# ml-jku/LaM-SLidE

Measured on AMD Instinct MI355X. Metric: sampled trajectories/sec (50-step ODE) + decoded-coord L2 vs ref, MD17, higher is better.
Workload: dtype bf16; 1 GPU; md17_bench; tail=False, ln_fuse=True, T=30, L=256, C=32, D=512, H=16, depth=4, sampler=ODE, state_updates=50, batch_per_gpu=32, global_batch=32, parallelism=batch-shard x1, 1 gather to rank 0 per step, noise_elem_stride_per_rank=7864320, kernels=general, trajectories_per_pass=32

## Files before the change

### lam_slide_amd/csrc/common.hip.h

```cpp
#pragma once
#include <hip/hip_runtime.h>
#include <stdint.h>

typedef unsigned short u16;
typedef __attribute__((ext_vector_type(8))) __bf16 bf16x8;
typedef __attribute__((ext_vector_type(4))) __bf16 bf16x4;
typedef __attribute__((ext_vector_type(16))) float f32x16;
typedef __attribute__((ext_vector_type(4))) short s16x4;
typedef __attribute__((ext_vector_type(4))) unsigned int u32x4;
typedef __attribute__((ext_vector_type(2))) unsigned int u32x2;

#define LDS_PTR(T) __attribute__((address_space(3))) T *

#define LSL_PROBE(v, bit) ((v) & (bit))

template <int N>
__device__ __forceinline__ void wait_vmcnt() { asm volatile("s_waitcnt vmcnt(%0)" ::"n"(N) : "memory"); }

__device__ __forceinline__ const char *uni_ptr(const char *q) {
    const unsigned long long v = (unsigned long long)q;
    const unsigned lo32 = __builtin_amdgcn_readfirstlane((unsigned)v), hi32 = __builtin_amdgcn_readfirstlane((unsigned)(v >> 32));
    return reinterpret_cast<const char *>(((unsigned long long)hi32 << 32) | lo32);
}
__device__ __forceinline__ void lds_dma16(unsigned voff, const void *base, unsigned dst) {
    asm volatile("s_mov_b32 m0, %2\n\ts_nop 4\n\tglobal_load_lds_dwordx4 %0, %1" ::"v"(voff), "s"(base), "s"(dst) : "memory");
}

__device__ __forceinline__ f32x16 mfma32(bf16x8 a, bf16x8 b, f32x16 c) {
    return __builtin_amdgcn_mfma_f32_32x32x16_bf16(a, b, c, 0, 0, 0);
}

__device__ __forceinline__ int acc_row(int reg, int hf) { return (reg & 3) + 8 * (reg >> 2) + 4 * hf; }

__device__ __forceinline__ u16 f2bf(float f) {
    __bf16 b = (__bf16)f;
    return __builtin_bit_cast(u16, b);
}
__device__ __forceinline__ float bf2f(u16 v) { return __uint_as_float(((unsigned)v) << 16); }

typedef __attribute__((ext_vector_type(2))) __bf16 bf16x2;
typedef __attribute__((ext_vector_type(2))) float f32x2;
__device__ __forceinline__ unsigned pack2(float lo, float hi) {
    const f32x2 v = {lo, hi};
    return __builtin_bit_cast(unsigned, __builtin_convertvector(v, bf16x2));
}

__device__ __forceinline__ bf16x8 as_bf16x8(u32x4 v) { return __builtin_bit_cast(bf16x8, v); }
__device__ __forceinline__ u32x4 as_u32x4(bf16x8 v) { return __builtin_bit_cast(u32x4, v); }

__device__ __forceinline__ float wave_sum(float v) {
#pragma unroll
    for (int o = 32; o > 0; o >>= 1) v += __shfl_xor(v, o, 64);
    return v;
}

#define LSL_DPP_ADD(v, ctrl, rows) ((v) + __builtin_bit_cast(float, __builtin_amdgcn_update_dpp(0, __builtin_bit_cast(int, (v)), (ctrl), (rows), 0xF, false)))
__device__ __forceinline__ float wave_sum_dpp(float v) {
    v = LSL_DPP_ADD(v, 0x111, 0xF);
    v = LSL_DPP_ADD(v, 0x112, 0xF);
    v = LSL_DPP_ADD(v, 0x114, 0xF);
    v = LSL_DPP_ADD(v, 0x118, 0xF);
    v = LSL_DPP_ADD(v, 0x142, 0xA);
    v = LSL_DPP_ADD(v, 0x143, 0xC);
    return __builtin_bit_cast(float, __builtin_amdgcn_readlane(__builtin_bit_cast(int, v), 63));
}
#undef LSL_DPP_ADD

__device__ __forceinline__ float xhalf(float v) { return __shfl_xor(v, 32, 64); }

__device__ __forceinline__ float half_pair_sum(float v) {
    const unsigned u = __builtin_bit_cast(unsigned, v);
    const auto p = __builtin_amdgcn_permlane32_swap(u, u, false, false);
    return __builtin_bit_cast(float, (unsigned)p[0]) + __builtin_bit_cast(float, (unsigned)p[1]);
}

__device__ __forceinline__ float quad_xor1(float v) {
    return __builtin_bit_cast(float, __builtin_amdgcn_update_dpp(0, __builtin_bit_cast(int, v), 0xB1, 0xF, 0xF, true));
}
__device__ __forceinline__ float quad_xor2(float v) {
    return __builtin_bit_cast(float, __builtin_amdgcn_update_dpp(0, __builtin_bit_cast(int, v), 0x4E, 0xF, 0xF, true));
}

__device__ __forceinline__ float oct_sum(float v) {
    v += quad_xor1(v);
    v += quad_xor2(v);
    return v + __builtin_bit_cast(float, __builtin_amdgcn_update_dpp(0, __builtin_bit_cast(int, v), 0x141, 0xF, 0xF, true));
}

__device__ __forceinline__ float silu(float x) { return x / (1.0f + __expf(-x)); }

__device__ __forceinline__ float gelu_erf(float x) { return 0.5f * x * (1.0f + erff(x * 0.70710678118654752440f)); }

#define LSL_GELU_Q(ax)                                                                                                  \
    fmaf(fmaf(fmaf(fmaf(fmaf(-0.0004733090754598379f, (ax), 0.0070845563896000385f), (ax), -0.051827382296323776f), (ax), \
                   -0.4599924385547638f), (ax), -1.1507878303527832f), (ax), -1.000037670135498f)
__device__ __forceinline__ float gelu_fast(float x) {
    const float ax = fabsf(x);
    const float h = __builtin_amdgcn_exp2f(LSL_GELU_Q(ax));
    const float relu = __builtin_amdgcn_fmed3f(x, 0.0f, __builtin_inff());
    return fmaf(-ax, h, relu);
}

__device__ __forceinline__ unsigned gelu_pair_bf16(float x0, float x1) {
    const f32x2 x = {x0, x1};
    const f32x2 ax = __builtin_elementwise_abs(x);
    f32x2 q = f32x2{-0.0004733090754598379f, -0.0004733090754598379f};
    q = __builtin_elementwise_fma(q, ax, f32x2{0.0070845563896000385f, 0.0070845563896000385f});
    q = __builtin_elementwise_fma(q, ax, f32x2{-0.051827382296323776f, -0.051827382296323776f});
    q = __builtin_elementwise_fma(q, ax, f32x2{-0.4599924385547638f, -0.4599924385547638f});
    q = __builtin_elementwise_fma(q, ax, f32x2{-1.1507878303527832f, -1.1507878303527832f});
    q = __builtin_elementwise_fma(q, ax, f32x2{-1.000037670135498f, -1.000037670135498f});
    const f32x2 h = {__builtin_amdgcn_exp2f(q[0]), __builtin_amdgcn_exp2f(q[1])};
    const f32x2 relu = {__int_as_float(max(__float_as_int(x0), 0)), __int_as_float(max(__float_as_int(x1), 0))};
    const f32x2 r = __builtin_elementwise_fma(-ax, h, relu);
    return __builtin_bit_cast(unsigned, __builtin_convertvector(r, bf16x2));
}

__device__ __forceinline__ void store16(void *p, u32x4 v, bool nt) {
    if (nt) asm volatile("global_store_dwordx4 %0, %1, off nt\n\ts_nop 1" ::"v"(p), "v"(v) : "memory");
    else *reinterpret_cast<u32x4 *>(p) = v;
}
__device__ __forceinline__ void store8(void *p, u32x2 v, bool nt) {
    if (nt) asm volatile("global_store_dwordx2 %0, %1, off nt\n\ts_nop 0" ::"v"(p), "v"(v) : "memory");
    else *reinterpret_cast<u32x2 *>(p) = v;
}

typedef __attribute__((ext_vector_type(4))) float f32x4_t;

__device__ __forceinline__ int xcd_remap(int bid, int nwg) {
    const int q = nwg >> 3, r = nwg & 7, xcd = bid & 7, idx = bid >> 3;
    const int base = xcd < r ? xcd * (q + 1) : r * (q + 1) + (xcd - r) * q;
    return base + idx;
}
```

### lam_slide_amd/csrc/k_lin1.hip.h

```cpp
#pragma once
#include <type_traits>

#include "common.hip.h"

struct Lin1Args {
    const u16 *W;
    const u16 *X;
    const float *bias;
    const float4 *rope_q, *rope_k;
    u16 *qkv;
    u16 *z;
    int F, N, HHD, M;
    int pos_div, pos_mod;
    unsigned div_magic, mod_magic;
    float inv_hd, q_premul;
    int nt;
    int wpt;
    int planes;
    int npad;
    const float2 *ln_stat;
    const float *ln_shift, *ln_scale;
    int ln_mod_stride, ln_tpt;
    unsigned ln_tpt_magic;
};

#ifndef LIN1_B2
#define LIN1_B2 1
#endif
#ifndef LIN1_B2_KMAX
#define LIN1_B2_KMAX 256
#endif

template <int HDP, int K, int NW = 8>
struct Lin1Cfg {
    static_assert(K % 128 == 0 && K <= 512, "hidden sizes 128 / 256 / 384 / 512");
    static constexpr int KS = K / 16;
    static constexpr int ROWB = 2 * K;
    static constexpr int PITCH = ROWB + 16;
    static constexpr int BLK = 32 * PITCH;
    static constexpr int NS = (LIN1_B2 && K <= LIN1_B2_KMAX) ? 4 : 3;
    static constexpr int RING = NS * BLK;
    static_assert(NW == 8 || NW == 4, "two waves per SIMD (256-token tiles) or one (128-token tiles)");
    static constexpr int TT = 32 * NW;
    static constexpr int STAGE = NW * 4096;
    static constexpr int LPR = ROWB / 16;
    static constexpr int PPW = 32 / NW;
    static constexpr size_t lds_bytes(int F) { return (size_t)RING + STAGE + (size_t)F * 4; }
    static constexpr int LN_SLOTS = K <= 256 ? 3 : 2;
    static constexpr size_t lds_bytes_lnf(int F) { return lds_bytes(F) + (size_t)LN_SLOTS * 2 * K * 4; }
};

enum { LIN1_QK = 0, LIN1_V = 1, LIN1_MLP = 2 };

#ifndef LIN1_XLOAD
#define LIN1_XLOAD 1
#endif
#ifndef LIN1_PD
#define LIN1_PD 3
#endif

__device__ __forceinline__ float lin1_gelu(float x) {
    const float ax = fabsf(x);
    const float h = __builtin_amdgcn_exp2f(LSL_GELU_Q(ax));
    float relu;
    asm("v_max_f32 %0, 0, %1" : "=v"(relu) : "v"(x));
    return fmaf(-ax, h, relu);
}

template <int HDP, int K, int NW = 8, bool LNF = false>
__global__ void __launch_bounds__(NW * 64, NW / 4) k_linear1_ts(Lin1Args g) {
    using C = Lin1Cfg<HDP, K, NW>;
    constexpr int KS = C::KS, BLK = C::BLK, PPW = C::PPW, ROWB = C::ROWB;
    constexpr int NCO = HDP == 32 ? 8 : 4;
    extern __shared__ __attribute__((aligned(16))) char smem[];

    const int tid = threadIdx.x, lane = tid & 63;
    const int wave = __builtin_amdgcn_readfirstlane(tid >> 6);
    const int r = lane & 31, hf = lane >> 5;
    char *const stage = smem + C::RING + wave * 4096;
    float *const bias_lds = reinterpret_cast<float *>(smem + C::RING + C::STAGE);

    const int NB = g.F >> 5;
    const int ntile = (g.N + C::TT - 1) / C::TT;
    const long U = (long)ntile * NB;
    long i0, i1;
    if (g.wpt > 0) {
        const int tile = blockIdx.x / g.wpt, part = blockIdx.x - tile * g.wpt;
        i0 = (long)tile * NB + ((NB * part / g.wpt) & ~1);
        i1 = (long)tile * NB + (part + 1 == g.wpt ? NB : ((NB * (part + 1) / g.wpt) & ~1));
    } else {
        i0 = (U * blockIdx.x / gridDim.x) & ~1L;
        i1 = blockIdx.x + 1 == gridDim.x ? U : ((U * (blockIdx.x + 1) / gridDim.x) & ~1L);
    }
    if (i0 >= i1) return;

    for (int i = tid * 4; i < g.F; i += NW * 64 * 4) *reinterpret_cast<float4 *>(bias_lds + i) = *reinterpret_cast<const float4 *>(g.bias + i);

    const unsigned lds0 = (unsigned)(size_t)(LDS_PTR(char))(smem);
    const unsigned lane_src = lane * 16;
    const char *const w_rows = reinterpret_cast<const char *>(g.W) + (size_t)(PPW * wave) * ROWB;
    auto issue_piece = [&](const char *src, unsigned dst, auto ic) __attribute__((always_inline)) {
        constexpr int I = decltype(ic)::value & 3;
        if (decltype(ic)::value >= 4) {
            src += 4 * ROWB;
            dst += 4 * C::PITCH;
        }
        const unsigned ls = lane_src;
        if (C::LPR == 64 || lane < C::LPR) {
            if (I == 0 || decltype(ic)::value >= 4)
                asm volatile("s_add_u32 m0, %2, %3\n\ts_nop 4\n\tglobal_load_lds_dwordx4 %0, %1 offset:%4" ::"v"(ls), "s"(src), "s"(dst), "n"(16 * I), "n"(ROWB * I) : "memory", "scc");
            else
                asm volatile("s_add_u32 m0, %2, %3\n\ts_nop 0\n\tglobal_load_lds_dwordx4 %0, %1 offset:%4" ::"v"(ls), "s"(src), "s"(dst), "n"(16 * I), "n"(ROWB * I) : "memory", "scc");
        }
    };
    auto req_src = [&](int blk) __attribute__((always_inline)) { return w_rows + (size_t)blk * (32 * ROWB); };
    auto req_dst = [&](int slot) __attribute__((always_inline)) { return lds0 + slot * BLK + PPW * wave * C::PITCH; };
    auto issue = [&](int blk, int slot) __attribute__((always_inline)) {
        const char *src = req_src(blk);
        const unsigned dst = req_dst(slot);
        issue_piece(src, dst, std::integral_constant<int, 0>());
        issue_piece(src, dst, std::integral_constant<int, 1>());
        issue_piece(src, dst, std::integral_constant<int, 2>());
        issue_piece(src, dst, std::integral_constant<int, 3>());
        if (PPW == 8) {
            issue_piece(src, dst, std::integral_constant<int, 4>());
            issue_piece(src, dst, std::integral_constant<int, 5>());
            issue_piece(src, dst, std::integral_constant<int, 6>());
            issue_piece(src, dst, std::integral_constant<int, 7>());
        }
    };
    const int aoff = r * C::PITCH + 16 * hf;

    bf16x8 xreg[KS];
    float4 co[NCO];
    f32x16 acc0, acc1;
    int slot_c = 0;
    int dma_blk, dma_slot;
    int n_wave = 0;
    float post = 1.0f;

    auto advance = [&](int &b) __attribute__((always_inline)) { b = b + 1 == NB ? 0 : b + 1; };
    auto next_slot = [&](int s) __attribute__((always_inline)) { return s == C::NS - 1 ? 0 : s + 1; };

    {
        int b = (int)(i0 - (i0 / NB) * NB);
        issue(b, 0);
        advance(b);
        issue(b, 1);
        advance(b);
        dma_blk = b;
        dma_slot = 2;
    }

    auto init_acc = [&](f32x16 &a, int blk) __attribute__((always_inline)) {
#pragma unroll
        for (int q4 = 0; q4 < 4; ++q4) {
            const float4 b = *reinterpret_cast<const float4 *>(bias_lds + blk * 32 + 8 * q4 + 4 * hf);
            a[4 * q4] = b.x; a[4 * q4 + 1] = b.y; a[4 * q4 + 2] = b.z; a[4 * q4 + 3] = b.w;
        }
    };
    constexpr bool B2 = LIN1_B2 != 0 && K <= LIN1_B2_KMAX;
    auto step_head = [&](auto flushed_c) __attribute__((always_inline)) {
        if (B2) {
            if (decltype(flushed_c)::value) wait_vmcnt<PPW>();
            else wait_vmcnt<0>();
        } else {
            if (decltype(flushed_c)::value) wait_vmcnt<2 * PPW>();
            else wait_vmcnt<PPW>();
        }
        __builtin_amdgcn_s_barrier();
        asm volatile("" ::: "memory");
    };
    const unsigned wr0 = (unsigned)(size_t)(LDS_PTR(char))(stage) + r * 128 + 8 * hf + ((r & 7) << 4);
    const unsigned rd0 = (unsigned)(size_t)(LDS_PTR(char))(stage) + (lane >> 3) * 128 + (((lane & 7) ^ ((lane >> 3) & 7)) << 4);
    const char *row_q = nullptr, *row_z = nullptr;
    const bool planes = g.planes != 0;
    constexpr unsigned PROW = 2u * HDP, CPH = HDP / 8;
    const unsigned plane_bytes = PROW * (unsigned)g.npad;
    const unsigned stride_q = planes ? PROW : 2u * 3 * g.HHD, stride_z = 2u * (g.HHD + g.M);
    const unsigned blk_q = planes ? (32 / HDP) * plane_bytes : 64u;
    const unsigned voff_q = planes ? ((lane & 7) / CPH) * plane_bytes + (lane >> 3) * PROW + 16 * ((lane & 7) % CPH) : (lane >> 3) * stride_q + 16 * (lane & 7);
    const unsigned voff_z = (lane >> 3) * stride_z + 16 * (lane & 7);
    const int slab_z = 3 * (g.HHD >> 5);
    const char *fl_base = nullptr;
    unsigned fl_stride8 = 0, fl_voff = 0;
    auto flush_setup = [&](int b_even) __attribute__((always_inline)) {
        const bool to_qkv = b_even < slab_z;
        fl_base = to_qkv ? row_q : row_z;
        fl_stride8 = 8 * (to_qkv ? stride_q : stride_z);
        fl_voff = to_qkv ? voff_q + blk_q * (unsigned)b_even : voff_z + 64u * (unsigned)b_even;
    };
    auto flush_read = [&](int half, u32x4 (&pk)[2]) __attribute__((always_inline)) {
#pragma unroll
        for (int i = 0; i < 2; ++i) pk[i] = *reinterpret_cast<const LDS_PTR(u32x4)>(rd0 + 1024 * (2 * half + i));
    };
    auto flush_store = [&](int half, const u32x4 (&pk)[2]) __attribute__((always_inline)) {
        asm volatile("s_nop 4\n\tglobal_store_dwordx4 %0, %1, %2 nt\n\ts_nop 1" ::"v"(fl_voff + (2 * half) * fl_stride8), "v"(pk[0]), "s"(fl_base) : "memory");
        asm volatile("global_store_dwordx4 %0, %1, %2 nt\n\ts_nop 1" ::"v"(fl_voff + (2 * half + 1) * fl_stride8), "v"(pk[1]), "s"(fl_base) : "memory");
    };
    auto flush_store_visible = [&](int half, const u32x4 (&pk)[2]) __attribute__((always_inline)) {
#pragma unroll
        for (int i = 0; i < 2; ++i)
            __builtin_nontemporal_store(pk[i], reinterpret_cast<u32x4 *>(const_cast<char *>(fl_base) + (size_t)(fl_voff + (2 * half + i) * fl_stride8)));
    };
    auto put_group = [&](int ii, int q, float v0, float v1, float v2, float v3) __attribute__((always_inline)) {
        const u32x2 pk = {pack2(v0, v1), pack2(v2, v3)};
        *reinterpret_cast<LDS_PTR(u32x2)>(wr0 ^ (unsigned)(64 * ii + 16 * q)) = pk;
    };
    auto epi_slice = [&](auto sec_c, int s, const f32x16 &a, int ii, float &c0, float &c1) __attribute__((always_inline)) {
        constexpr int SEC = decltype(sec_c)::value;
        if constexpr (SEC == LIN1_QK && HDP == 32) {
            if (s == 0) c0 = 0.0f;
            if (s < 2) {
#pragma unroll
                for (int e = 0; e < 8; ++e) c0 = fmaf(a[8 * s + e], a[8 * s + e], c0);
            }
            if (s == 1) c0 = rsqrtf(fmaf(half_pair_sum(c0), g.inv_hd, 1e-6f)) * post;
            if (s >= 2 && s < 6) {
                const int q = s - 2;
                float o[4];
#pragma unroll
                for (int kk = 0; kk < 2; ++kk) {
                    const int k = 2 * q + kk;
                    const float x0 = a[2 * k], x1 = a[2 * k + 1];
                    o[2 * kk] = c0 * fmaf(co[k].x, x0, -co[k].y * x1);
                    o[2 * kk + 1] = c0 * fmaf(co[k].z, x0, co[k].w * x1);
                }
                put_group(ii, q, o[0], o[1], o[2], o[3]);
            }
        } else if constexpr (SEC == LIN1_QK) {
            if (s == 0) {
                c0 = 0.0f;
#pragma unroll
                for (int e = 0; e < 8; ++e) c0 = fmaf(a[e], a[e], c0);
            }
            if (s == 1) {
                c1 = 0.0f;
#pragma unroll
                for (int e = 0; e < 8; ++e) c1 = fmaf(a[8 + e], a[8 + e], c1);
                c0 = rsqrtf(fmaf(half_pair_sum(c0), g.inv_hd, 1e-6f)) * post;
                c1 = rsqrtf(fmaf(half_pair_sum(c1), g.inv_hd, 1e-6f)) * post;
            }
            if (s >= 2 && s < 6) {
                const int q = s - 2;
                const float rr = q < 2 ? c0 : c1;
                float o[4];
#pragma unroll
                for (int kk = 0; kk < 2; ++kk) {
                    const int k = 2 * q + kk;
                    const float x0 = a[2 * k], x1 = a[2 * k + 1];
                    const float4 cf = co[k & (NCO - 1)];
                    o[2 * kk] = rr * fmaf(cf.x, x0, -cf.y * x1);
                    o[2 * kk + 1] = rr * fmaf(cf.z, x0, cf.w * x1);
                }
                put_group(ii, q, o[0], o[1], o[2], o[3]);
            }
        } else if constexpr (SEC == LIN1_MLP) {
            const float g0 = lin1_gelu(a[2 * s]), g1 = lin1_gelu(a[2 * s + 1]);
            if (s & 1) put_group(ii, s >> 1, c0, c1, g0, g1);
            else { c0 = g0; c1 = g1; }
        } else {
            if (s < 4) put_group(ii, s, a[4 * s], a[4 * s + 1], a[4 * s + 2], a[4 * s + 3]);
        }
    };
    auto step = [&](auto sec_c, auto par_c, auto mfma_c, auto epi_c, auto side) __attribute__((always_inline)) {
        constexpr int PAR = decltype(par_c)::value;
        constexpr bool DO_MFMA = decltype(mfma_c)::value != 0, DO_EPI = decltype(epi_c)::value != 0;
        constexpr int MPS = KS / 8, PD = LIN1_PD, MH = (MPS + 1) / 2;
        f32x16 &ac = PAR ? acc0 : acc1;
        const f32x16 &ae = PAR ? acc1 : acc0;
        const char *sb = smem + slot_c * BLK + aoff;
        bf16x8 fr[PD];
        float c0 = 0.0f, c1 = 0.0f;
        if (DO_MFMA) {
#pragma unroll
            for (int ks = 0; ks < PD; ++ks) fr[ks] = as_bf16x8(*reinterpret_cast<const u32x4 *>(sb + 32 * ks));
        }
        side(std::integral_constant<int, -1>());
#define LIN1_SIDE(S) if (s == S) side(std::integral_constant<int, S>());
#pragma unroll
        for (int s = 0; s < 8; ++s) {
#pragma unroll
            for (int m = 0; m < MPS; ++m) {
                if (m == MH) { LIN1_SIDE(0) LIN1_SIDE(1) LIN1_SIDE(2) LIN1_SIDE(3) LIN1_SIDE(4) LIN1_SIDE(5) LIN1_SIDE(6) LIN1_SIDE(7) }
                if (DO_MFMA) {
                    const int ks = s * MPS + m;
                    ac = mfma32(fr[ks % PD], xreg[ks], ac);
                    if (ks + PD < KS) fr[ks % PD] = as_bf16x8(*reinterpret_cast<const u32x4 *>(sb + 32 * (ks + PD)));
                }
            }
            if (MH == MPS) { LIN1_SIDE(0) LIN1_SIDE(1) LIN1_SIDE(2) LIN1_SIDE(3) LIN1_SIDE(4) LIN1_SIDE(5) LIN1_SIDE(6) LIN1_SIDE(7) }
            if (DO_EPI) epi_slice(sec_c, s, ae, PAR, c0, c1);
            __builtin_amdgcn_sched_barrier(0);
        }
#undef LIN1_SIDE
        if (decltype(mfma_c)::value != 0) slot_c = next_slot(slot_c);
    };
    std::integral_constant<int, 0> I0;
    std::integral_constant<int, 1> I1;
    auto no_side = [](auto) __attribute__((always_inline)) {};
    auto fused = [&](auto sec_c, auto par_c, auto flush_c, auto prev_c, int e) __attribute__((always_inline)) {
        constexpr int PAR = decltype(par_c)::value;
        constexpr bool FLUSH = decltype(flush_c)::value != 0;
        if (!B2 || PAR == 1) step_head(prev_c);
        u32x4 pk[2];
        if (FLUSH) flush_setup(e - 2);
        const char *src = req_src(dma_blk);
        const unsigned dst = req_dst(dma_slot);
        int blk2 = dma_blk;
        advance(blk2);
        const char *src2 = req_src(blk2);
        const unsigned dst2 = req_dst(next_slot(dma_slot));
        init_acc(PAR ? acc0 : acc1, e + 1);
        step(sec_c, par_c, I1, I1, [&](auto sl) __attribute__((always_inline)) {
            constexpr int SL = decltype(sl)::value;
            if (FLUSH) {
                if (SL == -1) flush_read(0, pk);
                if (SL == 0) {
                    flush_store(0, pk);
                    flush_read(1, pk);
                }
                if (SL == 1) flush_store(1, pk);
            }
            constexpr int PS = PPW / 4;
            if (!B2) {
                if (SL >= 2 && SL < 6) {
                    issue_piece(src, dst, std::integral_constant<int, (SL >= 2 && SL < 6) ? PS * (SL - 2) : 0>());
                    if (PS == 2) issue_piece(src, dst, std::integral_constant<int, (SL >= 2 && SL < 6) ? PS * (SL - 2) + 1 : 0>());
                }
            } else if (PAR == 1) {
                if (SL >= 0 && SL < 4) {
                    issue_piece(src, dst, std::integral_constant<int, (SL >= 0 && SL < 4) ? PS * SL : 0>());
                    if (PS == 2) issue_piece(src, dst, std::integral_constant<int, (SL >= 0 && SL < 4) ? PS * SL + 1 : 0>());
                }
                if (SL >= 4 && SL < 8) {
                    issue_piece(src2, dst2, std::integral_constant<int, (SL >= 4 && SL < 8) ? PS * (SL - 4) : 0>());
                    if (PS == 2) issue_piece(src2, dst2, std::integral_constant<int, (SL >= 4 && SL < 8) ? PS * (SL - 4) + 1 : 0>());
                }
            }
        });
        if (!B2) {
            advance(dma_blk);
            dma_slot = next_slot(dma_slot);
        } else if (PAR == 1) {
            advance(dma_blk);
            advance(dma_blk);
            dma_slot = next_slot(next_slot(dma_slot));
        }
    };
    auto run = [&](auto sec_c, int ea, int eb) __attribute__((always_inline)) {
        int e = ea;
        if (e < eb && (e & 1)) {
            fused(sec_c, I1, I0, I0, e);
            ++e;
        }
        for (; e + 1 < eb; e += 2) {
            fused(sec_c, I0, I1, I0, e);
            fused(sec_c, I1, I0, I1, e + 1);
        }
        if (e < eb) fused(sec_c, I0, I1, I0, e);
    };
    auto load_co = [&](const float4 *tab, unsigned pos) __attribute__((always_inline)) {
        const float4 *t = tab + (size_t)pos * (HDP / 2) + 2 * hf;
#pragma unroll
        for (int k = 0; k < NCO; ++k) co[k] = t[4 * (k >> 1) + (k & 1)];
    };
    std::integral_constant<int, LIN1_QK> SQK;
    std::integral_constant<int, LIN1_V> SV;
    std::integral_constant<int, LIN1_MLP> SMLP;

    constexpr bool XLINES = LIN1_XLOAD != 0 && (K <= 384 || LIN1_XLOAD >= 2);
    auto load_x = [&](int nw) __attribute__((always_inline)) {
        if (!XLINES) {
            const u16 *xr = g.X + (size_t)(nw + r) * K + 8 * hf;
#pragma unroll
            for (int ks = 0; ks < KS; ++ks) xreg[ks] = as_bf16x8(*reinterpret_cast<const u32x4 *>(xr + 16 * ks));
        } else {
            const u16 *xr = g.X + (size_t)(nw + (lane >> 3)) * K + 8 * (lane & 7);
#pragma unroll
            for (int j = 0; j < KS / 4; ++j)
#pragma unroll
                for (int q = 0; q < 4; ++q) xreg[4 * j + q] = as_bf16x8(*reinterpret_cast<const u32x4 *>(xr + (size_t)(8 * q) * K + 64 * j));
        }
    };
    auto finish_x = [&]() __attribute__((always_inline)) {
        if (!XLINES) return;
        const unsigned t0 = lane >> 3;
        const unsigned xw = (unsigned)(size_t)(LDS_PTR(char))(stage) + t0 * 128;
        const unsigned xr0 = (unsigned)(size_t)(LDS_PTR(char))(stage) + r * 128;
#pragma unroll
        for (int j = 0; j < KS / 4; ++j) {
#pragma unroll
            for (int q = 0; q < 4; ++q)
                *reinterpret_cast<LDS_PTR(u32x4)>(xw + 1024 * q + ((((lane & 7) ^ ((t0 >> 1) + 4 * q)) & 7) << 4)) = as_u32x4(xreg[4 * j + q]);
#pragma unroll
            for (int m = 0; m < 4; ++m)
                xreg[4 * j + m] = as_bf16x8(*reinterpret_cast<const LDS_PTR(u32x4)>(xr0 + ((((2 * m + hf) ^ (r >> 1)) & 7) << 4)));
        }
    };

    float *const ln_tab = bias_lds + ((g.F + 3) & ~3);
    auto traj_of = [&](unsigned n) __attribute__((always_inline)) { return g.ln_tpt_magic ? __umulhi(n, g.ln_tpt_magic) : n; };
    auto load_x_lnf = [&](int tile_, int nw) __attribute__((always_inline)) {
        typedef __attribute__((ext_vector_type(4))) float f4;
        const float *xf = reinterpret_cast<const float *>(g.X);
        const unsigned t_first = g.ln_mod_stride ? traj_of((unsigned)(tile_ * C::TT)) : 0u;
        const unsigned t_last = g.ln_mod_stride ? traj_of((unsigned)(g.N - 1)) : 0u;
        for (int i = tid * 4; i < C::LN_SLOTS * K; i += NW * 64 * 4) {
            const int slot = i / K, col = i - slot * K;
            const size_t mo = (size_t)min(t_first + (unsigned)slot, t_last) * g.ln_mod_stride + col;
            const f4 sc = *reinterpret_cast<const f4 *>(g.ln_scale + mo), sh = *reinterpret_cast<const f4 *>(g.ln_shift + mo);
            *reinterpret_cast<f4 *>(ln_tab + (size_t)slot * 2 * K + col) = f4{1.0f + sc[0], 1.0f + sc[1], 1.0f + sc[2], 1.0f + sc[3]};
            *reinterpret_cast<f4 *>(ln_tab + (size_t)slot * 2 * K + K + col) = sh;
        }
        const unsigned rowi = lane >> 3, chunk = lane & 7;
        const unsigned sbase = (unsigned)(size_t)(LDS_PTR(char))(stage);
        const unsigned xr0 = sbase + r * 128;
        const float *xr = xf + (size_t)(nw + rowi) * K + 4 * chunk;
        float2 st[4];
        const float *tb[4];
#pragma unroll
        for (int q = 0; q < 4; ++q) {
            const unsigned nn = (unsigned)min(nw + (int)rowi + 8 * q, g.N - 1);
            st[q] = g.ln_stat[nn];
            const unsigned slot = g.ln_mod_stride ? min(traj_of(nn) - t_first, (unsigned)(C::LN_SLOTS - 1)) : 0u;
            tb[q] = ln_tab + (size_t)slot * 2 * K + 4 * chunk;
        }
        __syncthreads();
#pragma unroll
        for (int p = 0; p < K / 64; ++p) {
            f4 v[2][4];
#pragma unroll
            for (int e = 0; e < 2; ++e)
#pragma unroll
                for (int q = 0; q < 4; ++q) v[e][q] = *reinterpret_cast<const f4 *>(xr + (size_t)(8 * q) * K + 64 * p + 32 * e);
#pragma unroll
            for (int q = 0; q < 4; ++q) {
                const unsigned row = rowi + 8 * q, sw = (row >> 1) & 7;
#pragma unroll
                for (int e = 0; e < 2; ++e) {
                    const f4 sc = *reinterpret_cast<const f4 *>(tb[q] + 64 * p + 32 * e), sh = *reinterpret_cast<const f4 *>(tb[q] + K + 64 * p + 32 * e);
                    f4 x = v[e][q];
#pragma unroll
                    for (int c = 0; c < 4; ++c) x[c] = fmaf(x[c], st[q].x, st[q].y) * sc[c] + sh[c];
                    const u32x2 pk = {pack2(x[0], x[1]), pack2(x[2], x[3])};
                    *reinterpret_cast<LDS_PTR(u32x2)>(sbase + row * 128 + ((((4 * e + (chunk >> 1)) ^ sw) & 7) << 4) + 8 * (chunk & 1)) = pk;
                }
            }
#pragma unroll
            for (int m = 0; m < 4; ++m)
                xreg[4 * p + m] = as_bf16x8(*reinterpret_cast<const LDS_PTR(u32x4)>(xr0 + ((((2 * m + hf) ^ (r >> 1)) & 7) << 4)));
            __builtin_amdgcn_sched_barrier(0);
        }
    };
    const int qb = g.HHD >> 5;
    int tile = (int)(i0 / NB), b0 = (int)(i0 - (long)tile * NB), left = (int)(i1 - i0);
    bool first_seg = true;
    bool co_ready = false;
    __syncthreads();
    while (left > 0) {
        const int b1 = NB - b0 < left ? NB : b0 + left;
        n_wave = tile * C::TT + wave * 32;
        row_q = reinterpret_cast<const char *>(g.qkv) + (size_t)n_wave * stride_q;
        row_z = reinterpret_cast<const char *>(g.z) + (size_t)n_wave * stride_z - 4 * (size_t)g.HHD;
        if constexpr (LNF) load_x_lnf(tile, n_wave);
        else {
            if (first_seg) load_x(n_wave);
            finish_x();
        }
        const unsigned nn = (unsigned)min(n_wave + r, g.N - 1);
        const unsigned n1 = g.div_magic ? __umulhi(nn, g.div_magic) : nn;
        const unsigned pos = g.mod_magic ? n1 - __umulhi(n1, g.mod_magic) * (unsigned)g.pos_mod : 0u;

        if (first_seg) wait_vmcnt<0>();
        else wait_vmcnt<4>();
        __builtin_amdgcn_s_barrier();
        asm volatile("" ::: "memory");
        issue(dma_blk, dma_slot);
        advance(dma_blk);
        dma_slot = next_slot(dma_slot);
        if (B2) {
            issue(dma_blk, dma_slot);
            advance(dma_blk);
            dma_slot = next_slot(dma_slot);
        }
        init_acc(acc0, b0);
        step(SV, I1, I1, I0, no_side);
        const int e_end = b1 - 1;
        if (b0 < 2 * qb) {
            if (!co_ready) load_co(b0 < qb ? g.rope_q : g.rope_k, pos);
            post = b0 < qb ? g.q_premul : 1.0f;
            fused(SQK, I0, I0, I0, b0);
        } else if (b0 < 3 * qb) {
            fused(SV, I0, I0, I0, b0);
        } else {
            fused(SMLP, I0, I0, I0, b0);
        }
        {
            const int lo = max(b0 + 1, 0), hi = min(e_end, qb);
            if (lo < hi) run(SQK, lo, hi);
        }
        {
            const int lo = max(b0 + 1, qb), hi = min(e_end, 2 * qb);
            if (lo < hi) {
                if (lo == qb) {
                    load_co(g.rope_k, pos);
                    post = 1.0f;
                }
                run(SQK, lo, hi);
            }
        }
        {
            const int lo = max(b0 + 1, 2 * qb), hi = min(e_end, 3 * qb);
            if (lo < hi) run(SV, lo, hi);
        }
        {
            const int lo = max(b0 + 1, 3 * qb), hi = min(e_end, NB);
            if (lo < hi) run(SMLP, lo, hi);
        }
        const int left_next = left - (b1 - b0);
        co_ready = false;
        if (left_next > 0) {
            asm volatile("" ::: "memory");
            const int nw = (tile + 1) * C::TT + wave * 32;
            if constexpr (!LNF) load_x(nw);
            if (b1 - 1 >= 2 * qb) {
                const unsigned nn2 = (unsigned)min(nw + r, g.N - 1);
                const unsigned m1 = g.div_magic ? __umulhi(nn2, g.div_magic) : nn2;
                load_co(g.rope_q, g.mod_magic ? m1 - __umulhi(m1, g.mod_magic) * (unsigned)g.pos_mod : 0u);
                co_ready = true;
            }
            asm volatile("" ::: "memory");
        }
        {
            const int e = b1 - 1;
            if (e < 2 * qb) {
                step(SQK, I1, I0, I1, no_side);
            } else if (e < 3 * qb) {
                step(SV, I1, I0, I1, no_side);
            } else {
                step(SMLP, I1, I0, I1, no_side);
            }
            flush_setup(e - 1);
            u32x4 pk[2];
            flush_read(0, pk);
            flush_store_visible(0, pk);
            flush_read(1, pk);
            flush_store_visible(1, pk);
        }
        left = left_next;
        tile += 1;
        b0 = 0;
        first_seg = false;
    }
    wait_vmcnt<0>();
}
```

Baseline: 58.10 trajectories/s.

## Recompute lane-derived addresses on demand and async-load RoPE tables via counted vmcnt waits

Replaces persistent per-lane address registers (aoff, wr0, rd0, voff_q/z, lane_src) with values recomputed from a fresh mbcnt lane id when K>=384 with 8 waves, aiming to lower VGPR pressure. RoPE cos/sin table loads become raw asm global loads that are issued early and consumed through explicit vmcnt waits folded into the step barrier, and the K-table switch is given its own fused step with a delayed wait. It also always prefetches the next tile's q table. The risk is extra ALU work for recomputation, and the hand-counted vmcnt values may be fragile.

After: 58.00 trajectories/s. No clear change (-0.2%).

```diff
diff --git a/lam_slide_amd/csrc/common.hip.h b/lam_slide_amd/csrc/common.hip.h
--- a/lam_slide_amd/csrc/common.hip.h
+++ b/lam_slide_amd/csrc/common.hip.h
@@ -16,6 +16,12 @@
 
 template <int N>
 __device__ __forceinline__ void wait_vmcnt() { asm volatile("s_waitcnt vmcnt(%0)" ::"n"(N) : "memory"); }
+
+__device__ __forceinline__ int fresh_lane_id() {
+    int l;
+    asm volatile("v_mbcnt_lo_u32_b32 %0, -1, 0\n\tv_mbcnt_hi_u32_b32 %0, -1, %0" : "=v"(l));
+    return l;
+}
 
 __device__ __forceinline__ const char *uni_ptr(const char *q) {
     const unsigned long long v = (unsigned long long)q;
diff --git a/lam_slide_amd/csrc/k_lin1.hip.h b/lam_slide_amd/csrc/k_lin1.hip.h
--- a/lam_slide_amd/csrc/k_lin1.hip.h
+++ b/lam_slide_amd/csrc/k_lin1.hip.h
@@ -72,6 +72,7 @@
     using C = Lin1Cfg<HDP, K, NW>;
     constexpr int KS = C::KS, BLK = C::BLK, PPW = C::PPW, ROWB = C::ROWB;
     constexpr int NCO = HDP == 32 ? 8 : 4;
+    constexpr bool RELANE = NW == 8 && K >= 384;
     extern __shared__ __attribute__((aligned(16))) char smem[];
 
     const int tid = threadIdx.x, lane = tid & 63;
@@ -97,7 +98,7 @@
     for (int i = tid * 4; i < g.F; i += NW * 64 * 4) *reinterpret_cast<float4 *>(bias_lds + i) = *reinterpret_cast<const float4 *>(g.bias + i);
 
     const unsigned lds0 = (unsigned)(size_t)(LDS_PTR(char))(smem);
-    const unsigned lane_src = lane * 16;
+    auto fresh_lane = [&]() __attribute__((always_inline)) { return RELANE ? fresh_lane_id() : lane; };
     const char *const w_rows = reinterpret_cast<const char *>(g.W) + (size_t)(PPW * wave) * ROWB;
     auto issue_piece = [&](const char *src, unsigned dst, auto ic) __attribute__((always_inline)) {
         constexpr int I = decltype(ic)::value & 3;
@@ -105,8 +106,9 @@
             src += 4 * ROWB;
             dst += 4 * C::PITCH;
         }
-        const unsigned ls = lane_src;
-        if (C::LPR == 64 || lane < C::LPR) {
+        const int l = fresh_lane();
+        const unsigned ls = l * 16;
+        if (C::LPR == 64 || l < C::LPR) {
             if (I == 0 || decltype(ic)::value >= 4)
                 asm volatile("s_add_u32 m0, %2, %3\n\ts_nop 4\n\tglobal_load_lds_dwordx4 %0, %1 offset:%4" ::"v"(ls), "s"(src), "s"(dst), "n"(16 * I), "n"(ROWB * I) : "memory", "scc");
             else
@@ -129,16 +131,30 @@
             issue_piece(src, dst, std::integral_constant<int, 7>());
         }
     };
-    const int aoff = r * C::PITCH + 16 * hf;
+    auto aoff_of = [&](int l) __attribute__((always_inline)) { return (l & 31) * C::PITCH + 16 * (l >> 5); };
 
     bf16x8 xreg[KS];
-    float4 co[NCO];
+    typedef __attribute__((ext_vector_type(4))) float co_t;
+    co_t co[NCO];
     f32x16 acc0, acc1;
     int slot_c = 0;
     int dma_blk, dma_slot;
     int n_wave = 0;
     float post = 1.0f;
 
+    auto bind_co = [&]() __attribute__((always_inline)) {
+        if constexpr (NCO == 8) asm volatile("" : "+v"(co[0]), "+v"(co[1]), "+v"(co[2]), "+v"(co[3]), "+v"(co[4]), "+v"(co[5]), "+v"(co[6]), "+v"(co[7]));
+        else asm volatile("" : "+v"(co[0]), "+v"(co[1]), "+v"(co[2]), "+v"(co[3]));
+    };
+    auto rot_pair = [&](const co_t &c, float rr, float x0, float x1, float &o0, float &o1) __attribute__((always_inline)) {
+        float t0, t1;
+        asm("v_mul_f32 %0, %1, %2" : "=v"(t0) : "v"(c.y), "v"(x1));
+        asm("v_fma_f32 %0, %1, %2, -%3" : "=v"(t0) : "v"(c.x), "v"(x0), "v"(t0));
+        asm("v_mul_f32 %0, %1, %2" : "=v"(o0) : "v"(rr), "v"(t0));
+        asm("v_mul_f32 %0, %1, %2" : "=v"(t1) : "v"(c.w), "v"(x1));
+        asm("v_fma_f32 %0, %1, %2, %3" : "=v"(t1) : "v"(c.z), "v"(x0), "v"(t1));
+        asm("v_mul_f32 %0, %1, %2" : "=v"(o1) : "v"(rr), "v"(t1));
+    };
     auto advance = [&](int &b) __attribute__((always_inline)) { b = b + 1 == NB ? 0 : b + 1; };
     auto next_slot = [&](int s) __attribute__((always_inline)) { return s == C::NS - 1 ? 0 : s + 1; };
 
@@ -153,6 +169,7 @@
     }
 
     auto init_acc = [&](f32x16 &a, int blk) __attribute__((always_inline)) {
+        const int hf = fresh_lane() >> 5;
 #pragma unroll
         for (int q4 = 0; q4 < 4; ++q4) {
             const float4 b = *reinterpret_cast<const float4 *>(bias_lds + blk * 32 + 8 * q4 + 4 * hf);
@@ -160,37 +177,43 @@
         }
     };
     constexpr bool B2 = LIN1_B2 != 0 && K <= LIN1_B2_KMAX;
-    auto step_head = [&](auto flushed_c) __attribute__((always_inline)) {
+    auto step_head = [&](auto flushed_c, auto extra_c) __attribute__((always_inline)) {
+        constexpr int EXTRA = decltype(extra_c)::value;
         if (B2) {
-            if (decltype(flushed_c)::value) wait_vmcnt<PPW>();
-            else wait_vmcnt<0>();
+            if (decltype(flushed_c)::value) wait_vmcnt<PPW + EXTRA>();
+            else wait_vmcnt<EXTRA>();
         } else {
-            if (decltype(flushed_c)::value) wait_vmcnt<2 * PPW>();
-            else wait_vmcnt<PPW>();
+            if (decltype(flushed_c)::value) wait_vmcnt<2 * PPW + EXTRA>();
+            else wait_vmcnt<PPW + EXTRA>();
         }
         __builtin_amdgcn_s_barrier();
         asm volatile("" ::: "memory");
     };
-    const unsigned wr0 = (unsigned)(size_t)(LDS_PTR(char))(stage) + r * 128 + 8 * hf + ((r & 7) << 4);
-    const unsigned rd0 = (unsigned)(size_t)(LDS_PTR(char))(stage) + (lane >> 3) * 128 + (((lane & 7) ^ ((lane >> 3) & 7)) << 4);
+    const unsigned stage0 = (unsigned)(size_t)(LDS_PTR(char))(stage);
+    auto wr0_of = [&](int l) __attribute__((always_inline)) { return stage0 + (l & 31) * 128 + 8 * (l >> 5) + ((l & 7) << 4); };
+    auto rd0_of = [&](int l) __attribute__((always_inline)) { return stage0 + (l >> 3) * 128 + (((l & 7) ^ ((l >> 3) & 7)) << 4); };
     const char *row_q = nullptr, *row_z = nullptr;
     const bool planes = g.planes != 0;
     constexpr unsigned PROW = 2u * HDP, CPH = HDP / 8;
     const unsigned plane_bytes = PROW * (unsigned)g.npad;
     const unsigned stride_q = planes ? PROW : 2u * 3 * g.HHD, stride_z = 2u * (g.HHD + g.M);
     const unsigned blk_q = planes ? (32 / HDP) * plane_bytes : 64u;
-    const unsigned voff_q = planes ? ((lane & 7) / CPH) * plane_bytes + (lane >> 3) * PROW + 16 * ((lane & 7) % CPH) : (lane >> 3) * stride_q + 16 * (lane & 7);
-    const unsigned voff_z = (lane >> 3) * stride_z + 16 * (lane & 7);
+    auto voff_q_of = [&](unsigned l) __attribute__((always_inline)) {
+        return planes ? ((l & 7) / CPH) * plane_bytes + (l >> 3) * PROW + 16 * ((l & 7) % CPH) : (l >> 3) * stride_q + 16 * (l & 7);
+    };
+    auto voff_z_of = [&](unsigned l) __attribute__((always_inline)) { return (l >> 3) * stride_z + 16 * (l & 7); };
     const int slab_z = 3 * (g.HHD >> 5);
     const char *fl_base = nullptr;
     unsigned fl_stride8 = 0, fl_voff = 0;
     auto flush_setup = [&](int b_even) __attribute__((always_inline)) {
         const bool to_qkv = b_even < slab_z;
+        const unsigned l = (unsigned)fresh_lane();
         fl_base = to_qkv ? row_q : row_z;
         fl_stride8 = 8 * (to_qkv ? stride_q : stride_z);
-        fl_voff = to_qkv ? voff_q + blk_q * (unsigned)b_even : voff_z + 64u * (unsigned)b_even;
+        fl_voff = to_qkv ? voff_q_of(l) + blk_q * (unsigned)b_even : voff_z_of(l) + 64u * (unsigned)b_even;
     };
     auto flush_read = [&](int half, u32x4 (&pk)[2]) __attribute__((always_inline)) {
+        const unsigned rd0 = rd0_of(fresh_lane());
 #pragma unroll
         for (int i = 0; i < 2; ++i) pk[i] = *reinterpret_cast<const LDS_PTR(u32x4)>(rd0 + 1024 * (2 * half + i));
     };
@@ -203,11 +226,11 @@
         for (int i = 0; i < 2; ++i)
             __builtin_nontemporal_store(pk[i], reinterpret_cast<u32x4 *>(const_cast<char *>(fl_base) + (size_t)(fl_voff + (2 * half + i) * fl_stride8)));
     };
-    auto put_group = [&](int ii, int q, float v0, float v1, float v2, float v3) __attribute__((always_inline)) {
+    auto put_group = [&](unsigned wr0, int ii, int q, float v0, float v1, float v2, float v3) __attribute__((always_inline)) {
         const u32x2 pk = {pack2(v0, v1), pack2(v2, v3)};
         *reinterpret_cast<LDS_PTR(u32x2)>(wr0 ^ (unsigned)(64 * ii + 16 * q)) = pk;
     };
-    auto epi_slice = [&](auto sec_c, int s, const f32x16 &a, int ii, float &c0, float &c1) __attribute__((always_inline)) {
+    auto epi_slice = [&](auto sec_c, int s, const f32x16 &a, int ii, unsigned wr0, float &c0, float &c1) __attribute__((always_inline)) {
         constexpr int SEC = decltype(sec_c)::value;
         if constexpr (SEC == LIN1_QK && HDP == 32) {
             if (s == 0) c0 = 0.0f;
@@ -223,10 +246,9 @@
                 for (int kk = 0; kk < 2; ++kk) {
                     const int k = 2 * q + kk;
                     const float x0 = a[2 * k], x1 = a[2 * k + 1];
-                    o[2 * kk] = c0 * fmaf(co[k].x, x0, -co[k].y * x1);
-                    o[2 * kk + 1] = c0 * fmaf(co[k].z, x0, co[k].w * x1);
-                }
-                put_group(ii, q, o[0], o[1], o[2], o[3]);
+                    rot_pair(co[k], c0, x0, x1, o[2 * kk], o[2 * kk + 1]);
+                }
+                put_group(wr0, ii, q, o[0], o[1], o[2], o[3]);
             }
         } else if constexpr (SEC == LIN1_QK) {
             if (s == 0) {
@@ -249,27 +271,27 @@
                 for (int kk = 0; kk < 2; ++kk) {
                     const int k = 2 * q + kk;
                     const float x0 = a[2 * k], x1 = a[2 * k + 1];
-                    const float4 cf = co[k & (NCO - 1)];
-                    o[2 * kk] = rr * fmaf(cf.x, x0, -cf.y * x1);
-                    o[2 * kk + 1] = rr * fmaf(cf.z, x0, cf.w * x1);
-                }
-                put_group(ii, q, o[0], o[1], o[2], o[3]);
+                    rot_pair(co[k & (NCO - 1)], rr, x0, x1, o[2 * kk], o[2 * kk + 1]);
+                }
+                put_group(wr0, ii, q, o[0], o[1], o[2], o[3]);
             }
         } else if constexpr (SEC == LIN1_MLP) {
             const float g0 = lin1_gelu(a[2 * s]), g1 = lin1_gelu(a[2 * s + 1]);
-            if (s & 1) put_group(ii, s >> 1, c0, c1, g0, g1);
+            if (s & 1) put_group(wr0, ii, s >> 1, c0, c1, g0, g1);
             else { c0 = g0; c1 = g1; }
         } else {
-            if (s < 4) put_group(ii, s, a[4 * s], a[4 * s + 1], a[4 * s + 2], a[4 * s + 3]);
-        }
-    };
-    auto step = [&](auto sec_c, auto par_c, auto mfma_c, auto epi_c, auto side) __attribute__((always_inline)) {
+            if (s < 4) put_group(wr0, ii, s, a[4 * s], a[4 * s + 1], a[4 * s + 2], a[4 * s + 3]);
+        }
+    };
+    auto step = [&](auto sec_c, auto par_c, auto mfma_c, auto epi_c, auto side, auto co_wait) __attribute__((always_inline)) {
         constexpr int PAR = decltype(par_c)::value;
         constexpr bool DO_MFMA = decltype(mfma_c)::value != 0, DO_EPI = decltype(epi_c)::value != 0;
         constexpr int MPS = KS / 8, PD = LIN1_PD, MH = (MPS + 1) / 2;
         f32x16 &ac = PAR ? acc0 : acc1;
         const f32x16 &ae = PAR ? acc1 : acc0;
-        const char *sb = smem + slot_c * BLK + aoff;
+        const int l = fresh_lane();
+        const char *sb = smem + slot_c * BLK + aoff_of(l);
+        const unsigned wr0 = wr0_of(l);
         bf16x8 fr[PD];
         float c0 = 0.0f, c1 = 0.0f;
         if (DO_MFMA) {
@@ -290,7 +312,8 @@
                 }
             }
             if (MH == MPS) { LIN1_SIDE(0) LIN1_SIDE(1) LIN1_SIDE(2) LIN1_SIDE(3) LIN1_SIDE(4) LIN1_SIDE(5) LIN1_SIDE(6) LIN1_SIDE(7) }
-            if (DO_EPI) epi_slice(sec_c, s, ae, PAR, c0, c1);
+            if (DO_EPI && s == 2) co_wait();
+            if (DO_EPI) epi_slice(sec_c, s, ae, PAR, wr0, c0, c1);
             __builtin_amdgcn_sched_barrier(0);
         }
 #undef LIN1_SIDE
@@ -299,10 +322,12 @@
     std::integral_constant<int, 0> I0;
     std::integral_constant<int, 1> I1;
     auto no_side = [](auto) __attribute__((always_inline)) {};
-    auto fused = [&](auto sec_c, auto par_c, auto flush_c, auto prev_c, int e) __attribute__((always_inline)) {
+    auto no_wait = []() __attribute__((always_inline)) {};
+    auto fused = [&](auto sec_c, auto par_c, auto flush_c, auto prev_c, auto co_c, int e) __attribute__((always_inline)) {
         constexpr int PAR = decltype(par_c)::value;
-        constexpr bool FLUSH = decltype(flush_c)::value != 0;
-        if (!B2 || PAR == 1) step_head(prev_c);
+        constexpr bool FLUSH = decltype(flush_c)::value != 0, CO = decltype(co_c)::value != 0;
+        static_assert(!CO || PAR == 0, "the table rows are requested in front of an even step");
+        if (!B2 || PAR == 1) step_head(prev_c, std::integral_constant<int, CO ? NCO : 0>());
         u32x4 pk[2];
         if (FLUSH) flush_setup(e - 2);
         const char *src = req_src(dma_blk);
@@ -338,6 +363,11 @@
                     if (PS == 2) issue_piece(src2, dst2, std::integral_constant<int, (SL >= 4 && SL < 8) ? PS * (SL - 4) + 1 : 0>());
                 }
             }
+        }, [&]() __attribute__((always_inline)) {
+            if (CO) {
+                wait_vmcnt<(FLUSH ? 4 : 0) + (B2 ? 0 : PPW / 4)>();
+                bind_co();
+            }
         });
         if (!B2) {
             advance(dma_blk);
@@ -348,22 +378,29 @@
             dma_slot = next_slot(next_slot(dma_slot));
         }
     };
-    auto run = [&](auto sec_c, int ea, int eb) __attribute__((always_inline)) {
+    auto run = [&](auto sec_c, int ea, int eb, auto first_prev_c) __attribute__((always_inline)) {
         int e = ea;
         if (e < eb && (e & 1)) {
-            fused(sec_c, I1, I0, I0, e);
+            fused(sec_c, I1, I0, first_prev_c, I0, e);
             ++e;
         }
         for (; e + 1 < eb; e += 2) {
-            fused(sec_c, I0, I1, I0, e);
-            fused(sec_c, I1, I0, I1, e + 1);
-        }
-        if (e < eb) fused(sec_c, I0, I1, I0, e);
-    };
-    auto load_co = [&](const float4 *tab, unsigned pos) __attribute__((always_inline)) {
-        const float4 *t = tab + (size_t)pos * (HDP / 2) + 2 * hf;
-#pragma unroll
-        for (int k = 0; k < NCO; ++k) co[k] = t[4 * (k >> 1) + (k & 1)];
+            fused(sec_c, I0, I1, I0, I0, e);
+            fused(sec_c, I1, I0, I1, I0, e + 1);
+        }
+        if (e < eb) fused(sec_c, I0, I1, I0, I0, e);
+    };
+    auto load_co = [&](const float4 *tab, int nw) __attribute__((always_inline)) {
+        const int l = fresh_lane();
+        const unsigned nn = (unsigned)min(nw + (l & 31), g.N - 1);
+        const unsigned n1 = g.div_magic ? __umulhi(nn, g.div_magic) : nn;
+        const unsigned pos = g.mod_magic ? n1 - __umulhi(n1, g.mod_magic) * (unsigned)g.pos_mod : 0u;
+        const unsigned off = (pos * (unsigned)(HDP / 2) + 2u * (unsigned)(l >> 5)) * 16u;
+#pragma unroll
+        for (int k = 0; k < NCO; ++k) {
+            if (k == 0) asm volatile("s_nop 4\n\tglobal_load_dwordx4 %0, %1, %2 offset:%3" : "=&v"(co[k]) : "v"(off), "s"(tab), "n"(16 * (4 * (k >> 1) + (k & 1))) : "memory");
+            else asm volatile("global_load_dwordx4 %0, %1, %2 offset:%3" : "=&v"(co[k]) : "v"(off), "s"(tab), "n"(16 * (4 * (k >> 1) + (k & 1))) : "memory");
+        }
     };
     std::integral_constant<int, LIN1_QK> SQK;
     std::integral_constant<int, LIN1_V> SV;
@@ -371,6 +408,7 @@
 
     constexpr bool XLINES = LIN1_XLOAD != 0 && (K <= 384 || LIN1_XLOAD >= 2);
     auto load_x = [&](int nw) __attribute__((always_inline)) {
+        const int lane = fresh_lane(), r = lane & 31, hf = lane >> 5;
         if (!XLINES) {
             const u16 *xr = g.X + (size_t)(nw + r) * K + 8 * hf;
 #pragma unroll
@@ -385,6 +423,7 @@
     };
     auto finish_x = [&]() __attribute__((always_inline)) {
         if (!XLINES) return;
+        const int lane = fresh_lane(), r = lane & 31, hf = lane >> 5;
         const unsigned t0 = lane >> 3;
         const unsigned xw = (unsigned)(size_t)(LDS_PTR(char))(stage) + t0 * 128;
         const unsigned xr0 = (unsigned)(size_t)(LDS_PTR(char))(stage) + r * 128;
@@ -413,18 +452,19 @@
             *reinterpret_cast<f4 *>(ln_tab + (size_t)slot * 2 * K + col) = f4{1.0f + sc[0], 1.0f + sc[1], 1.0f + sc[2], 1.0f + sc[3]};
             *reinterpret_cast<f4 *>(ln_tab + (size_t)slot * 2 * K + K + col) = sh;
         }
+        const int lane = fresh_lane(), r = lane & 31, hf = lane >> 5;
         const unsigned rowi = lane >> 3, chunk = lane & 7;
-        const unsigned sbase = (unsigned)(size_t)(LDS_PTR(char))(stage);
+        const unsigned sbase = stage0;
         const unsigned xr0 = sbase + r * 128;
         const float *xr = xf + (size_t)(nw + rowi) * K + 4 * chunk;
         float2 st[4];
-        const float *tb[4];
+        unsigned tb[4];
 #pragma unroll
         for (int q = 0; q < 4; ++q) {
             const unsigned nn = (unsigned)min(nw + (int)rowi + 8 * q, g.N - 1);
             st[q] = g.ln_stat[nn];
             const unsigned slot = g.ln_mod_stride ? min(traj_of(nn) - t_first, (unsigned)(C::LN_SLOTS - 1)) : 0u;
-            tb[q] = ln_tab + (size_t)slot * 2 * K + 4 * chunk;
+            tb[q] = slot * 2 * K + 4 * chunk;
         }
         __syncthreads();
 #pragma unroll
@@ -439,7 +479,7 @@
                 const unsigned row = rowi + 8 * q, sw = (row >> 1) & 7;
 #pragma unroll
                 for (int e = 0; e < 2; ++e) {
-                    const f4 sc = *reinterpret_cast<const f4 *>(tb[q] + 64 * p + 32 * e), sh = *reinterpret_cast<const f4 *>(tb[q] + K + 64 * p + 32 * e);
+                    const f4 sc = *reinterpret_cast<const f4 *>(ln_tab + tb[q] + 64 * p + 32 * e), sh = *reinterpret_cast<const f4 *>(ln_tab + tb[q] + K + 64 * p + 32 * e);
                     f4 x = v[e][q];
 #pragma unroll
                     for (int c = 0; c < 4; ++c) x[c] = fmaf(x[c], st[q].x, st[q].y) * sc[c] + sh[c];
@@ -456,24 +496,25 @@
     const int qb = g.HHD >> 5;
     int tile = (int)(i0 / NB), b0 = (int)(i0 - (long)tile * NB), left = (int)(i1 - i0);
     bool first_seg = true;
-    bool co_ready = false;
     __syncthreads();
     while (left > 0) {
         const int b1 = NB - b0 < left ? NB : b0 + left;
         n_wave = tile * C::TT + wave * 32;
         row_q = reinterpret_cast<const char *>(g.qkv) + (size_t)n_wave * stride_q;
         row_z = reinterpret_cast<const char *>(g.z) + (size_t)n_wave * stride_z - 4 * (size_t)g.HHD;
+        if (first_seg && b0 < 2 * qb) load_co(b0 < qb ? g.rope_q : g.rope_k, n_wave);
         if constexpr (LNF) load_x_lnf(tile, n_wave);
         else {
             if (first_seg) load_x(n_wave);
             finish_x();
         }
-        const unsigned nn = (unsigned)min(n_wave + r, g.N - 1);
-        const unsigned n1 = g.div_magic ? __umulhi(nn, g.div_magic) : nn;
-        const unsigned pos = g.mod_magic ? n1 - __umulhi(n1, g.mod_magic) * (unsigned)g.pos_mod : 0u;
-
-        if (first_seg) wait_vmcnt<0>();
-        else wait_vmcnt<4>();
+
+        if (first_seg) {
+            wait_vmcnt<0>();
+            bind_co();
+        } else {
+            wait_vmcnt<4>();
+        }
         __builtin_amdgcn_s_barrier();
         asm volatile("" ::: "memory");
         issue(dma_blk, dma_slot);
@@ -485,61 +526,57 @@
             dma_slot = next_slot(dma_slot);
         }
         init_acc(acc0, b0);
-        step(SV, I1, I1, I0, no_side);
+        step(SV, I1, I1, I0, no_side, no_wait);
         const int e_end = b1 - 1;
         if (b0 < 2 * qb) {
-            if (!co_ready) load_co(b0 < qb ? g.rope_q : g.rope_k, pos);
             post = b0 < qb ? g.q_premul : 1.0f;
-            fused(SQK, I0, I0, I0, b0);
+            fused(SQK, I0, I0, I0, I0, b0);
         } else if (b0 < 3 * qb) {
-            fused(SV, I0, I0, I0, b0);
+            fused(SV, I0, I0, I0, I0, b0);
         } else {
-            fused(SMLP, I0, I0, I0, b0);
+            fused(SMLP, I0, I0, I0, I0, b0);
         }
         {
             const int lo = max(b0 + 1, 0), hi = min(e_end, qb);
-            if (lo < hi) run(SQK, lo, hi);
+            if (lo < hi) run(SQK, lo, hi, I0);
         }
         {
             const int lo = max(b0 + 1, qb), hi = min(e_end, 2 * qb);
             if (lo < hi) {
                 if (lo == qb) {
-                    load_co(g.rope_k, pos);
+                    load_co(g.rope_k, n_wave);
                     post = 1.0f;
-                }
-                run(SQK, lo, hi);
+                    fused(SQK, I0, I1, I0, I1, lo);
+                    run(SQK, lo + 1, hi, I1);
+                } else {
+                    run(SQK, lo, hi, I0);
+                }
             }
         }
         {
             const int lo = max(b0 + 1, 2 * qb), hi = min(e_end, 3 * qb);
-            if (lo < hi) run(SV, lo, hi);
+            if (lo < hi) run(SV, lo, hi, I0);
         }
         {
             const int lo = max(b0 + 1, 3 * qb), hi = min(e_end, NB);
-            if (lo < hi) run(SMLP, lo, hi);
+            if (lo < hi) run(SMLP, lo, hi, I0);
         }
         const int left_next = left - (b1 - b0);
-        co_ready = false;
         if (left_next > 0) {
             asm volatile("" ::: "memory");
             const int nw = (tile + 1) * C::TT + wave * 32;
             if constexpr (!LNF) load_x(nw);
-            if (b1 - 1 >= 2 * qb) {
-                const unsigned nn2 = (unsigned)min(nw + r, g.N - 1);
-                const unsigned m1 = g.div_magic ? __umulhi(nn2, g.div_magic) : nn2;
-                load_co(g.rope_q, g.mod_magic ? m1 - __umulhi(m1, g.mod_magic) * (unsigned)g.pos_mod : 0u);
-                co_ready = true;
-            }
+            load_co(g.rope_q, nw);
             asm volatile("" ::: "memory");
         }
         {
             const int e = b1 - 1;
-            if (e < 2 * qb) {
-                step(SQK, I1, I0, I1, no_side);
+            if (left_next <= 0 && e < 2 * qb) {
+                step(SQK, I1, I0, I1, no_side, no_wait);
             } else if (e < 3 * qb) {
-                step(SV, I1, I0, I1, no_side);
+                step(SV, I1, I0, I1, no_side, no_wait);
             } else {
-                step(SMLP, I1, I0, I1, no_side);
+                step(SMLP, I1, I0, I1, no_side, no_wait);
             }
             flush_setup(e - 1);
             u32x4 pk[2];
@@ -547,6 +584,10 @@
             flush_store_visible(0, pk);
             flush_read(1, pk);
             flush_store_visible(1, pk);
+        }
+        if (left_next > 0) {
+            wait_vmcnt<4>();
+            bind_co();
         }
         left = left_next;
         tile += 1;
```
